# statgen/demuxlet

Measured on AMD Instinct MI355X. Metric: cell-SNP-sample triples/sec (singlet+doublet llk); HBM GB/s vs roofline, higher is better.
Workload: dtype f64

## Files before the change

demuxlet_amd/csrc/dmx_engine.hip:

```cpp
#include <hip/hip_runtime.h>

#include <algorithm>
#include <chrono>
#include <cmath>
#include <mutex>
#include <cstdlib>
#include <cstring>
#include <condition_variable>
#include <deque>
#include <new>
#include <memory>
#include <functional>
#include <thread>
#include <type_traits>
#include <unordered_map>
#include <cxxabi.h>
#include <string>
#include <numeric>
#include <vector>

#include "dmx_internal.hpp"
extern char** environ;
#include "dmx_log.hpp"
#include "dmx_engine_state.hpp"
// ... 3115 lines not shown
      DMX_WAVE_LDS_ORDER();
      const int cnt = (int)min<int64_t>(kTripPT, p_end - p0);
      for (int jj = 0; jj < cnt; jj += 2) {
        const int j = jj + h;
        const uint32_t nj = (ent && j < cnt) ? hdr[j].n : 0u;
        if (nj > 0) {
          const int64_t roff = hdr[j].off;
          uint32_t w = hdr[j].rd4;
          double f = s_pra[w & 0xFF][0] * qk + s_pra[w & 0xFF][1] * pk;
          int32_t E = 0;
          const bool deep = nj >= 8;
          for (uint32_t r = 1; r < nj; ++r) {
            if ((r & 3) == 0) w = load_rd4(pv, roff + r, nj - r);
            const uint32_t byte = (w >> (8 * (r & 3))) & 0xFF;
            f *= s_pra[byte][0] * qk + s_pra[byte][1] * pk;
            if (deep && (r & 7) == 7 && f < kAmbRescaleBelow && f > 0.0) {
              int e;
              (void)frexp(f, &e);
              f = ldexp(f, -e);
              E += e;
            }
          }
          const double wk = (double)hdr[j].gp[el] * (double)hdr[j].gp[3 + em];
          const double t = wk * f;
          st[j][k] = t;
          ste[j][k] = t > 0.0 ? E : kTripNoExp;
        }
      }
      DMX_WAVE_LDS_ORDER();
      if (fj < cnt && hdr[fj].n > 0) {
        int32_t En = kTripNoExp;
#pragma unroll
        for (int x = 0; x < 9; ++x) En = max(En, ste[fj][3 * x + fn]);
        if (En == kTripNoExp) En = 0;
        double u = 0.0;
#pragma unroll
        for (int x = 0; x < 9; ++x) {
          const double t = ldexp(st[fj][3 * x + fn], max(ste[fj][3 * x + fn] - En, -1100));
          u = x == 0 ? t : u + t;
        }
        su[fj][fn] = u;
        sue[fj][fn] = u > 0.0 ? En : kTripNoExp;
      }
      DMX_WAVE_LDS_ORDER();
      for (int j = 0; j < cnt; ++j) {
        const uint32_t nj = (uint32_t)__builtin_amdgcn_readfirstlane((int)hdr[j].n);
        if (nj == 0) continue;
        const int32_t snp = __builtin_amdgcn_readfirstlane(hdr[j].snp);
        const double u0 = amb_uniform(su[j][0]), u1 = amb_uniform(su[j][1]), u2 = amb_uniform(su[j][2]);
        const int32_t e0 = __builtin_amdgcn_readfirstlane(sue[j][0]), e1 = __builtin_amdgcn_readfirstlane(sue[j][1]),
                      e2 = __builtin_amdgcn_readfirstlane(sue[j][2]);
        const float* gs = g + (size_t)snp * V * 3;
#pragma unroll
        for (int a = 0; a < NACC; ++a) {
          const int32_t c = c0 + 64 * a;
          const float* gr = gs + (size_t)(c < V ? c : 0) * 3;
          const float g0 = gr[0], g1 = gr[1], g2 = gr[2];
          const bool nz = g0 != 0.f || g1 != 0.f || g2 != 0.f;
          double L;
          int32_t E = 0;
          if (nj < 8) {
            L = (double)g0 * u0 + (double)g1 * u1 + (double)g2 * u2;
          } else {
            E = kTripNoExp;
            if (g0 != 0.f) E = max(E, e0);
            if (g1 != 0.f) E = max(E, e1);
            if (g2 != 0.f) E = max(E, e2);
            if (E == kTripNoExp) E = 0;
            const double t0 = g0 != 0.f ? (double)g0 * ldexp(u0, max(e0 - E, -1100)) : 0.0;
            const double t1 = g1 != 0.f ? (double)g1 * ldexp(u1, max(e1 - E, -1100)) : 0.0;
            const double t2 = g2 != 0.f ? (double)g2 * ldexp(u2, max(e2 - E, -1100)) : 0.0;
            L = t0 + t1 + t2;
          }
          if (!nz) L = 1.0;
          double lg = dmx_log_is_special(L) ? log(L) : dmx_log_fast_pinned(L, s_log, lk);
          if (E != 0) lg = __builtin_fma((double)E, DMX_LOG_LN2HI, __builtin_fma((double)E, DMX_LOG_LN2LO, lg));
          if (nz) { acc[a] += lg; ns[a] += 1; nr[a] += (int32_t)nj; }
        }
      }
      DMX_WAVE_LDS_ORDER();
    }
  }
#pragma unroll
  for (int a = 0; a < NACC; ++a) {
    const int32_t c = c0 + 64 * a;
    if (c >= V) continue;
    ll[((size_t)slot * T + ti) * V + c] = acc[a];
    if (ti == 0) { n_snp[(size_t)slot * V + c] = ns[a]; n_read[(size_t)slot * V + c] = nr[a]; }
  }
}

__global__ void k_transpose_geno(const float* __restrict__ g, const double* __restrict__ gp0, int32_t S, int32_t V,
                                 float* __restrict__ gT, double* __restrict__ g0T) {
  const int nrow = V * 3;
  const int64_t n = (int64_t)S * nrow;
  for (int64_t i = (int64_t)blockIdx.x * blockDim.x + threadIdx.x; i < n; i += (int64_t)gridDim.x * blockDim.x) {
    const int64_t s = i % S;
    const int r = (int)(i / S);
    gT[i] = g[(size_t)s * nrow + r];
    if (r < 3) g0T[i] = gp0[(size_t)s * 3 + r];
  }
}

template <typename NRD, int NACC, bool FIXUP>
__global__ __launch_bounds__(kThreads) void k_doublet_generic(PileupView pv, const float* __restrict__ g,
                                                              const double* __restrict__ gp0,
                                                              const double* __restrict__ lut,
                                                              const double* __restrict__ alpha,
                                                              const int32_t* __restrict__ sched, int32_t V, int32_t A,
                                                              int32_t A_pad, int32_t TP, double* __restrict__ grid,
                                                              double* __restrict__ l00,
                                                              uint8_t* __restrict__ flagged) {
  if (FIXUP && !flags_any(flagged)) return;
  __shared__ double s_lut[kTab2];
  __shared__ double s_pG[kThreads * 9];
  __shared__ int32_t s_snp[32];
  __shared__ uint32_t s_cnt[32];
  __shared__ int64_t s_off[32];

  const int t = threadIdx.x;
  stage_k2_tables(s_lut, lut, t, kThreads);
  const double* s_log = s_lut + kLut2;
  for (int32_t bx = (int32_t)blockIdx.x; bx < pv.B; bx += (int32_t)gridDim.x) {
  if (FIXUP && !flagged[sched[bx]]) continue;
  const int32_t cell = sched[bx];
  const int64_t p_beg = pv.cell_pair_off[cell];
  const int64_t np = pv.cell_pair_off[cell + 1] - p_beg;
  int64_t rd_base = pv.cell_read_off[cell];
  const NRD* __restrict__ nrd = (const NRD*)pv.pair_nrd;

  const int ti1 = t / A_pad, n1 = t % A_pad;
  const bool lane1 = (ti1 < TP) && (n1 < A);
  double wA[9], wR[9];
  {
    const double al = lane1 ? alpha[n1] : 0.0;
#pragma unroll
    for (int l = 0; l < 3; ++l)
#pragma unroll
      for (int m = 0; m < 3; ++m) {
        const double p = 0.5 * l + (m - l) * 0.5 * al;
        wA[l * 3 + m] = p;
        wR[l * 3 + m] = 1.0 - p;
      }
  }

  const int32_t nAB = V * V * A;
  const int32_t nacc = nAB + A;
  const int32_t q0 = (int32_t)blockIdx.y * NACC * kThreads;
  bool ok = true;
  uint32_t code[NACC];
  double acc[NACC];
#pragma unroll
  for (int i = 0; i < NACC; ++i) {
    const int32_t q = q0 + t + i * kThreads;
    acc[i] = 0.0;
    if (q < nAB) {
      const int32_t n = q % A, jk = q / A;
      code[i] = ((uint32_t)(jk / V) << 20) | ((uint32_t)(jk % V) << 8) | (uint32_t)n;
    } else if (q < nacc) {
      code[i] = (0xFFFu << 20) | (uint32_t)(q - nAB);
    } else {
      code[i] = ~0u;
    }
  }
  __syncthreads();

  for (int64_t base = 0; base < np; base += TP) {
    const int tp = (int)min((int64_t)TP, np - base);
    if (t < 32) {
      const bool v = t < tp;
      const uint32_t n = v ? (uint32_t)nrd[p_beg + base + t] : 0u;
      uint32_t incl = n;
#pragma unroll
      for (int d = 1; d < 32; d <<= 1) {
        const uint32_t y = __shfl_up(incl, d, 32);
        if (t >= d) incl += y;
      }
      if (v) {
        s_cnt[t] = n;
        s_off[t] = rd_base + (int64_t)(incl - n);
        s_snp[t] = pv.pair_snp ? pv.pair_snp[p_beg + base + t] : (int32_t)(base + t);
      }
    }
    __syncthreads();
    rd_base = s_off[tp - 1] + (int64_t)s_cnt[tp - 1];

    {
      const bool on = lane1 && ti1 < tp;
      const uint32_t cnt = on ? s_cnt[ti1] : 0u;
      const int64_t off = on ? s_off[ti1] : 0;
      const uint32_t rd4 = load_rd4(pv, off, cnt);
      double pG[9];
      const double mx = pair_values_open<9, 0, true>(pv, cnt, off, rd4, s_lut, wA, wR, n1, pG, nullptr, on, A_pad);
      if (on) {
        const double y = rcp_refined(mx);
#pragma unroll
        for (int i = 0; i < 9; ++i) s_pG[(ti1 * A + n1) * 9 + i] = div_by(pG[i], mx, y);
      }
    }
    __syncthreads();

    for (int ti = 0; ti < tp; ++ti) {
      const int32_t snp = s_snp[ti];
      const float* __restrict__ grow = g + (size_t)snp * V * 3;
      const double* __restrict__ g0 = gp0 + (size_t)snp * 3;
#pragma unroll
      for (int i = 0; i < NACC; ++i) {
        const uint32_t cd = code[i];
        if (cd == ~0u) continue;
        const int32_t j = (cd >> 20) & 0xFFF, k = (cd >> 8) & 0xFFF, n = cd & 0xFF;
        double a[3], b[3];
        if (j == 0xFFF) {
          a[0] = b[0] = g0[0]; a[1] = b[1] = g0[1]; a[2] = b[2] = g0[2];
        } else {
          a[0] = (double)grow[j * 3]; a[1] = (double)grow[j * 3 + 1]; a[2] = (double)grow[j * 3 + 2];
          b[0] = (double)grow[k * 3]; b[1] = (double)grow[k * 3 + 1]; b[2] = (double)grow[k * 3 + 2];
        }
        const double* P = &s_pG[(ti * A + n) * 9];
        double sum = 0.0;
#pragma unroll
        for (int l = 0; l < 3; ++l)
#pragma unroll
          for (int m = 0; m < 3; ++m) sum += ((a[l] * b[m]) * P[l * 3 + m]);
        if (!FIXUP) ok &= __builtin_amdgcn_class(sum, 0x100);
        acc[i] += FIXUP ? log(sum) : dmx_log2_fast(sum, s_log);
      }
    }
    __syncthreads();
  }

#pragma unroll
  for (int i = 0; i < NACC; ++i) {
    const int32_t q = q0 + t + i * kThreads;
    if (q < nAB) grid[(size_t)cell * nAB + q] = acc[i];
    else if (q < nacc) l00[(size_t)cell * A + (q - nAB)] = acc[i];
  }
  if (!FIXUP && !ok) flag_cell(flagged, cell);
  __syncthreads();
  }
}

template <int TPC, int NK, int MINW, bool GD, bool CHK, int TP, bool SYMU>
__device__ __forceinline__ void a2_body(PileupView pv, int nrd_width, const float* __restrict__ g,
                                                         const double* __restrict__ gp0, const double* __restrict__ tabs,
                                                         const double* __restrict__ alpha,
                                                         const int32_t* __restrict__ sched, int32_t V, int32_t GS,
                                                         double* __restrict__ grid, double* __restrict__ l00,
                                                         uint8_t* __restrict__ flagged, const double* __restrict__ pfin, const double* __restrict__ pseed) {
  static_assert(!SYMU || ((TPC == 256 || TPC == 64) && NK == 4 && !CHK), "symmetric ownership: 32 samples on 256 threads or 16 on 64, eight accumulators per thread, provably safe rows");
  constexpr int kUV = TPC == 256 ? 32 : 16, kUSh = kUV == 32 ? 5 : 4;
  constexpr int A = 2;
  static_assert(TP == 32 || TP == 16 || TP == 8, "phase 1 runs on the first 2 * TP lanes of the cell's first wavefront");
  constexpr int CPW = kThreads / TPC;
  constexpr int T00 = TP + 2;
#define DMX_K2_SYNC() do { if (TPC == 64) { DMX_WAVE_LDS_ORDER(); } else { __syncthreads(); } } while (0)
  extern __shared__ __attribute__((aligned(16))) unsigned char s_raw[];
  __shared__ double s_tab[kTab2];
  __shared__ double s_w[2][18];
  const double* s_log = s_tab + kLut2;
  const int t = threadIdx.x;
  stage_k2_tables(s_tab, tabs, t, kThreads);
  if (t < 18) {
    const int n = t / 9, l = (t % 9) / 3, m = t % 3;
    const double p = 0.5 * l + (m - l) * 0.5 * alpha[n];
    s_w[n][t % 9] = p;
    s_w[n][9 + t % 9] = 1.0 - p;
  }
  __syncthreads();

  const int cw = t / TPC, tid = t % TPC;
  using g_t = typename std::conditional<GD, double, float>::type;
  const size_t cell_bytes = (size_t)TP * 18 * 8 + (size_t)TP * GS * sizeof(g_t) + 2 * T00 * 8 + TP * (4 + 4 + 8);
  unsigned char* base = s_raw + (size_t)cw * cell_bytes;
  double* s_pG = (double*)base;
  g_t* s_g = (g_t*)(base + (size_t)TP * 18 * 8);
  double* s_t00 = (double*)((unsigned char*)s_g + (size_t)TP * GS * sizeof(g_t));
  int64_t* s_off = (int64_t*)(s_t00 + 2 * T00);
  int32_t* s_snp = (int32_t*)(s_off + TP);
  uint32_t* s_cnt = (uint32_t*)(s_snp + TP);

  const int slot = blockIdx.x * CPW + cw;
  if (TPC == 64 && slot >= pv.B) return;
  const bool cell_ok = slot < pv.B;
  const int32_t cell = cell_ok ? sched[slot] : 0;
  const int64_t p_beg = cell_ok ? pv.cell_pair_off[cell] : 0;
  const int64_t np = cell_ok ? pv.cell_pair_off[cell + 1] - p_beg : 0;
  int64_t rd_base = cell_ok ? pv.cell_read_off[cell] : 0;

  const int KB = (V + NK - 1) / NK;
  const int JS = TPC / KB;
  const int jl = tid / KB, kb = tid % KB;
  const int j = (int)blockIdx.y * JS + jl;
  const bool owner = jl < JS && j < V;
  double acc[NK][A];
#pragma unroll
  for (int kk = 0; kk < NK; ++kk) { acc[kk][0] = 0.0; acc[kk][1] = 0.0; }
  bool ok = true;
  const DmxLogPins lk = dmx_log_pins();
  int uj[2] = {0, 0}, uk[2] = {0, 0};
  if constexpr (SYMU) {
#pragma unroll
    for (int su = 0; su < 2; ++su) { const int u = tid + TPC * su; uj[su] = u & (kUV - 1); uk[su] = (uj[su] + 1 + (u >> kUSh)) & (kUV - 1); }
  }
  const int ti1 = tid >> 1, n1 = tid & 1;
  double acc00 = 0.0;
  const int row_len = V * 3;

  for (int64_t tbase = 0; tbase < np; tbase += TP) {
    const int tp = (int)min((int64_t)TP, np - tbase);
    load_tile_headers<TP>(pv, nrd_width, p_beg, tbase, tp, tid, rd_base, s_cnt, s_off, s_snp);
    DMX_K2_SYNC();
    rd_base = s_off[tp - 1] + (int64_t)s_cnt[tp - 1];
    stage_geno_rows<TPC>(g, s_snp, tp, tid, row_len, GS, s_g);
    if (tid < 2 * TP) {
      const bool on = ti1 < tp;
      const uint32_t cnt = on ? s_cnt[ti1] : 0u;
      const int64_t off = on ? s_off[ti1] : 0;
      const uint32_t rd4 = load_rd4(pv, off, cnt);
      double vf[9];
      const int32_t fi = pfin ? certify_final_index(cnt, rd4) : -1;
      if (!__any(fi < 0)) {
        const double* fp = pfin + (size_t)fi * kCFinStride + (n1 ? 0 : 5);
        const double f0 = fp[0], f1 = fp[1], f2 = fp[2], f3 = n1 ? fp[3] : 0.0, f4 = n1 ? fp[4] : 0.0;
        const double f5[5] = {f0, f1, f2, f3, f4};
#pragma unroll
        for (int l = 0; l < 3; ++l)
#pragma unroll
          for (int m = 0; m < 3; ++m) vf[l * 3 + m] = n1 ? f5[l + m] : f5[l];
      } else if (pseed) {
        double q5[5], wA5[5], wR5[5];
#pragma unroll
        for (int q = 0; q < 5; ++q) {
          const int l = n1 ? (q > 2 ? 2 : q) : min(q, 2), m = n1 ? q - l : 0;
          const double p = 0.5 * l + (m - l) * 0.5 * (n1 ? 0.5 : 0.0);
          wA5[q] = p;
          wR5[q] = 1.0 - p;
        }
        certify_pair_values<5, false>(pv, cnt, off, rd4, s_tab, wA5, wR5, n1, q5, pseed);
#pragma unroll
        for (int l = 0; l < 3; ++l)
#pragma unroll
          for (int m = 0; m < 3; ++m) vf[l * 3 + m] = n1 ? q5[l + m] : q5[l];
      } else {
        double wA[9], wR[9];
#pragma unroll
        for (int i = 0; i < 9; ++i) { wA[i] = s_w[n1][i]; wR[i] = s_w[n1][9 + i]; }
        certify_pair_values<9, false, 2, true>(pv, cnt, off, rd4, s_tab, wA, wR, n1, vf);
      }
      if (on)
        ok &= llks00_term(gp0, s_snp[ti1], [&](int l, int m) { const double v = vf[l * 3 + m]; s_pG[(ti1 * 2 + n1) * 9 + l * 3 + m] = v; return v; },
                    s_log, &s_t00[n1 * T00 + ti1]);
    }
    DMX_K2_SYNC();
    if (tid < 2) {
      const double* row = &s_t00[tid * T00];
      if (tp == TP) {
        double2 v[TP / 2];
#pragma unroll
        for (int i = 0; i < TP / 2; ++i) v[i] = *reinterpret_cast<const double2*>(&row[2 * i]);
#pragma unroll
        for (int i = 0; i < TP / 2; ++i) { acc00 += v[i].x; acc00 += v[i].y; }
      } else {
        for (int i = 0; i < tp; ++i) acc00 += row[i];
      }
    }
    if constexpr (SYMU) {
      for (int ti = 0; ti < tp; ++ti) {
        const double* P = &s_pG[ti * 18];
        const double Q[3] = {P[0], P[3], P[6]};
        const double P1[5] = {P[9], P[10], P[11], P[14], P[17]};
        const g_t* gr = &s_g[ti * GS];
#pragma unroll
        for (int su = 0; su < 2; ++su) {
          const int js = uj[su], ks = uk[su];
          const double a[3] = {(double)gr[js * 3], (double)gr[js * 3 + 1], (double)gr[js * 3 + 2]};
          const double b[3] = {(double)gr[ks * 3], (double)gr[ks * 3 + 1], (double)gr[ks * 3 + 2]};
          double E[3][3];
#pragma unroll
          for (int l = 0; l < 3; ++l)
#pragma unroll
            for (int m = 0; m < 3; ++m) E[l][m] = a[l] * b[m];
          {
            double s_jk0 = E[0][0] * Q[0], s_kj0 = E[0][0] * Q[0];
#pragma unroll
            for (int l = 0; l < 3; ++l)
#pragma unroll
              for (int m = 0; m < 3; ++m) {
                if (l == 0 && m == 0) continue;
                s_jk0 += (E[l][m] * Q[l]);
                s_kj0 += (E[m][l] * Q[l]);
              }
            acc[2 * su][0] += dmx_log2_fast_pinned(s_jk0, s_log, lk);
            acc[2 * su + 1][0] += dmx_log2_fast_pinned(s_kj0, s_log, lk);
          }
          {
#pragma unroll
            for (int l = 0; l < 3; ++l)
#pragma unroll
              for (int m = 0; m < 3; ++m) E[l][m] = E[l][m] * P1[l + m];
            double s_jk1 = E[0][0], s_kj1 = E[0][0];
#pragma unroll
            for (int l = 0; l < 3; ++l)
#pragma unroll
              for (int m = 0; m < 3; ++m) {
                if (l == 0 && m == 0) continue;
                s_jk1 += E[l][m];
                s_kj1 += E[m][l];
              }
            acc[2 * su][1] += dmx_log2_fast_pinned(s_jk1, s_log, lk);
            acc[2 * su + 1][1] += dmx_log2_fast_pinned(s_kj1, s_log, lk);
          }
        }
      }
    } else
    if (owner) {
      for (int ti = 0; ti < tp; ++ti) {
        const double* P = &s_pG[ti * 18];
        double P0[9], P1[9];
#pragma unroll
        for (int i = 0; i < 9; ++i) { P0[i] = P[i]; P1[i] = P[9 + i]; }
        const g_t* gr = &s_g[ti * GS];
        const double a0 = (double)gr[j * 3], a1 = (double)gr[j * 3 + 1], a2 = (double)gr[j * 3 + 2];
        const double aj[3] = {a0, a1, a2};
#pragma unroll
        for (int kk = 0; kk < NK; ++kk) {
          const int k = min(kb * NK + kk, V - 1);
          const double b0 = (double)gr[k * 3], b1 = (double)gr[k * 3 + 1], b2 = (double)gr[k * 3 + 2];
          const double bk[3] = {b0, b1, b2};
          double s0 = (aj[0] * bk[0]) * P0[0], s1 = (aj[0] * bk[0]) * P1[0];
#pragma unroll
          for (int l = 0; l < 3; ++l)
#pragma unroll
            for (int m = 0; m < 3; ++m) {
              if (l == 0 && m == 0) continue;
              const double gp = aj[l] * bk[m];
              s0 += (gp * P0[l * 3 + m]);
              s1 += (gp * P1[l * 3 + m]);
            }
          if (CHK) ok &= __builtin_amdgcn_class(s0, 0x100) && __builtin_amdgcn_class(s1, 0x100);
          acc[kk][0] += dmx_log2_fast_pinned(s0, s_log, lk);
          acc[kk][1] += dmx_log2_fast_pinned(s1, s_log, lk);
        }
      }
    }
    DMX_K2_SYNC();
  }
  if (cell_ok) {
    if constexpr (SYMU) {
#pragma unroll
      for (int su = 0; su < 2; ++su) {
        const int u = tid + TPC * su, d = 1 + (u >> kUSh);
        if (d < kUV / 2 || (d == kUV / 2 && uj[su] < kUV / 2)) {
          double* o = grid + (((size_t)cell * V + uj[su]) * V + uk[su]) * A;
          o[0] = acc[2 * su][0]; o[1] = acc[2 * su][1];
          double* o2 = grid + (((size_t)cell * V + uk[su]) * V + uj[su]) * A;
          o2[0] = acc[2 * su + 1][0]; o2[1] = acc[2 * su + 1][1];
        }
      }
    } else
    if (owner) {
#pragma unroll
      for (int kk = 0; kk < NK; ++kk) {
        const int k = kb * NK + kk;
        if (k < V) {
          double* o = grid + (((size_t)cell * V + j) * V + k) * A;
          o[0] = acc[kk][0]; o[1] = acc[kk][1];
        }
      }
    }
    if (tid < 2 && blockIdx.y == 0) l00[(size_t)cell * A + tid] = acc00;
    if (!ok) flag_cell(flagged, cell);
  }
#undef DMX_K2_SYNC
}
template <int TPC, int NK, int MINW = 1, bool GD = false, bool CHK = true, int TP = 32>
__global__ __launch_bounds__(kThreads, (MINW == 1 && TPC == 64) ? 3 : MINW) void k_doublet_a2(PileupView pv, int nrd_width, const float* __restrict__ g,
                                                         const double* __restrict__ gp0, const double* __restrict__ tabs,
                                                         const double* __restrict__ alpha,
                                                         const int32_t* __restrict__ sched, int32_t V, int32_t GS,
                                                         double* __restrict__ grid, double* __restrict__ l00,
                                                         uint8_t* __restrict__ flagged, const double* __restrict__ pfin, const double* __restrict__ pseed) {
  a2_body<TPC, NK, MINW, GD, CHK, TP, false>(pv, nrd_width, g, gp0, tabs, alpha, sched, V, GS, grid, l00, flagged, pfin, pseed);
}
template <int MINW>
__global__ __launch_bounds__(kThreads, MINW) void k_doublet_a2u(PileupView pv, int nrd_width, const float* __restrict__ g,
                                                          const double* __restrict__ gp0, const double* __restrict__ tabs,
                                                          const double* __restrict__ alpha,
                                                          const int32_t* __restrict__ sched, int32_t V, int32_t GS,
                                                          double* __restrict__ grid, double* __restrict__ l00,
                                                          uint8_t* __restrict__ flagged, const double* __restrict__ pfin, const double* __restrict__ pseed) {
  a2_body<256, 4, MINW, true, false, 32, true>(pv, nrd_width, g, gp0, tabs, alpha, sched, V, GS, grid, l00, flagged, pfin, pseed);
}
__global__ __launch_bounds__(kThreads, 3) void k_doublet_a2u16(PileupView pv, int nrd_width, const float* __restrict__ g,
                                                          const double* __restrict__ gp0, const double* __restrict__ tabs,
                                                          const double* __restrict__ alpha,
                                                          const int32_t* __restrict__ sched, int32_t V, int32_t GS,
                                                          double* __restrict__ grid, double* __restrict__ l00,
                                                          uint8_t* __restrict__ flagged, const double* __restrict__ pfin, const double* __restrict__ pseed) {
  a2_body<64, 4, 1, false, false, 32, true>(pv, nrd_width, g, gp0, tabs, alpha, sched, V, GS, grid, l00, flagged, pfin, pseed);
}

template <int TPC, int NK>
__global__ __launch_bounds__(kThreads, 3) void k_doublet_a2f(PileupView pv, int nrd_width, const float* __restrict__ g,
                                                         const double* __restrict__ gp0, const double* __restrict__ tabs,
                                                         const double* __restrict__ alpha,
                                                         const int32_t* __restrict__ sched, int32_t V, int32_t GS,
                                                         double* __restrict__ grid, double* __restrict__ l00,
                                                         uint8_t* __restrict__ flagged) {
  constexpr int A = 2, TP = 32;
  constexpr int CPW = kThreads / TPC;
  constexpr int T00 = TP + 2;
#define DMX_K2_SYNC() do { if (TPC == 64) { DMX_WAVE_LDS_ORDER(); } else { __syncthreads(); } } while (0)
  extern __shared__ __attribute__((aligned(16))) unsigned char s_raw[];
  __shared__ double s_tab[kTab2];
  const double* s_log = s_tab + kLut2;
  const int t = threadIdx.x;
  stage_k2_tables(s_tab, tabs, t, kThreads);
  __syncthreads();

  const int cw = t / TPC, tid = t % TPC;
  constexpr bool SHARE = TPC > 64;
  constexpr int SUB = 8;
  const int VU = V;
  const size_t cell_bytes = (size_t)TP * 18 * 8 + (size_t)TP * GS * 4 + 2 * T00 * 8 + TP * (4 + 4 + 8) + (SHARE ? (size_t)SUB * 2 * VU * 32 : 0);
  unsigned char* base = s_raw + (size_t)cw * cell_bytes;
  double* s_pG = (double*)base;
  float* s_g = (float*)(base + (size_t)TP * 18 * 8);
  double* s_t00 = (double*)((unsigned char*)s_g + (size_t)TP * GS * 4);
  int64_t* s_off = (int64_t*)(s_t00 + 2 * T00);
  int32_t* s_snp = (int32_t*)(s_off + TP);
  uint32_t* s_cnt = (uint32_t*)(s_snp + TP);
  double* s_u = (double*)(s_cnt + TP);

  const int slot = blockIdx.x * CPW + cw;
  if (TPC == 64 && slot >= pv.B) return;
  const bool cell_ok = slot < pv.B;
  const int32_t cell = cell_ok ? sched[slot] : 0;
  const int64_t p_beg = cell_ok ? pv.cell_pair_off[cell] : 0;
  const int64_t np = cell_ok ? pv.cell_pair_off[cell + 1] - p_beg : 0;
  int64_t rd_base = cell_ok ? pv.cell_read_off[cell] : 0;

  const int KB = (V + NK - 1) / NK;
  const int JS = TPC / KB;
  const int jl = tid / KB, kb = tid % KB;
  const int j = (int)blockIdx.y * JS + jl;
  const bool owner = jl < JS && j < V;
  double acc[NK][A];
#pragma unroll
  for (int kk = 0; kk < NK; ++kk) { acc[kk][0] = 0.0; acc[kk][1] = 0.0; }
  bool ok = true;
  const DmxLogPins lk = dmx_log_pins();
  const int ti1 = tid >> 1, n1 = tid & 1;
  double wA[9], wR[9];
  {
    const double al = alpha[n1];
#pragma unroll
    for (int l = 0; l < 3; ++l)
#pragma unroll
      for (int m = 0; m < 3; ++m) {
        const double p = 0.5 * l + (m - l) * 0.5 * al;
        wA[l * 3 + m] = p;
        wR[l * 3 + m] = 1.0 - p;
      }
  }
  double acc00 = 0.0;
  const int row_len = V * 3;

  for (int64_t tbase = 0; tbase < np; tbase += TP) {
    const int tp = (int)min((int64_t)TP, np - tbase);
    load_tile_headers<TP>(pv, nrd_width, p_beg, tbase, tp, tid, rd_base, s_cnt, s_off, s_snp);
    DMX_K2_SYNC();
    rd_base = s_off[tp - 1] + (int64_t)s_cnt[tp - 1];
    stage_geno_rows<TPC>(g, s_snp, tp, tid, row_len, GS, s_g);
    if (tid < 64) {
      const bool on = ti1 < tp;
      const uint32_t cnt = on ? s_cnt[ti1] : 0u;
      const int64_t off = on ? s_off[ti1] : 0;
      const uint32_t rd4 = load_rd4(pv, off, cnt);
      double pG[9];
      const double mx = pair_values_open<9, 2, true>(pv, cnt, off, rd4, s_tab, wA, wR, n1, pG);
      if (on) {
        const double y = rcp_refined(mx);
        ok &= llks00_term(gp0, s_snp[ti1], [&](int l, int m) { const double v = div_by(pG[l * 3 + m], mx, y); s_pG[(ti1 * 2 + n1) * 9 + l * 3 + m] = v; return v; },
                    s_log, &s_t00[n1 * T00 + ti1]);
      }
    }
    DMX_K2_SYNC();
    if (tid < 2) {
      const double* row = &s_t00[tid * T00];
      if (tp == TP) {
        double2 v[TP / 2];
#pragma unroll
        for (int i = 0; i < TP / 2; ++i) v[i] = *reinterpret_cast<const double2*>(&row[2 * i]);
#pragma unroll
        for (int i = 0; i < TP / 2; ++i) { acc00 += v[i].x; acc00 += v[i].y; }
      } else {
        for (int i = 0; i < tp; ++i) acc00 += row[i];
      }
    }
    if (!SHARE) {
      if (owner) {
        for (int ti = 0; ti < tp; ++ti) {
          const double* P = &s_pG[ti * 18];
          double P0[9], P1[9];
#pragma unroll
          for (int i = 0; i < 9; ++i) { P0[i] = P[i]; P1[i] = P[9 + i]; }
          const float* gr = &s_g[ti * GS];
          const double a0 = (double)gr[j * 3], a1 = (double)gr[j * 3 + 1], a2 = (double)gr[j * 3 + 2];
#pragma unroll
          for (int kk = 0; kk < NK; ++kk) {
            const int k = min(kb * NK + kk, V - 1);
            const double b0 = (double)gr[k * 3], b1 = (double)gr[k * 3 + 1], b2 = (double)gr[k * 3 + 2];
            double x[3], y[3];
#pragma unroll
            for (int l = 0; l < 3; ++l) {
              x[l] = __builtin_fma(P0[l * 3 + 2], b2, __builtin_fma(P0[l * 3 + 1], b1, P0[l * 3] * b0));
              y[l] = __builtin_fma(P1[l * 3 + 2], b2, __builtin_fma(P1[l * 3 + 1], b1, P1[l * 3] * b0));
            }
            const double s0 = __builtin_fma(a2, x[2], __builtin_fma(a1, x[1], a0 * x[0]));
            const double s1 = __builtin_fma(a2, y[2], __builtin_fma(a1, y[1], a0 * y[0]));
            ok &= __builtin_amdgcn_class(s0, 0x100) && __builtin_amdgcn_class(s1, 0x100);
            acc[kk][0] += dmx_log2_fastmode(s0, s_log, lk);
            acc[kk][1] += dmx_log2_fastmode(s1, s_log, lk);
          }
        }
      }
      DMX_K2_SYNC();
    } else
#pragma unroll 1
    for (int sub = 0; sub < tp; sub += SUB) {
      const int ns = min(SUB, tp - sub);
#pragma unroll 1
      for (int e = tid; e < ns * 2 * V; e += TPC) {
        const int k = e % V, n = (e / V) & 1, pi = e / (2 * V);
        const double* P = &s_pG[((sub + pi) * 2 + n) * 9];
        const float* gr = &s_g[(sub + pi) * GS + k * 3];
        const double b0 = (double)gr[0], b1 = (double)gr[1], b2 = (double)gr[2];
        double* u = &s_u[(size_t)((pi * 2 + n) * VU + k) * 4];
#pragma unroll
        for (int l = 0; l < 3; ++l) u[l] = __builtin_fma(P[l * 3 + 2], b2, __builtin_fma(P[l * 3 + 1], b1, P[l * 3] * b0));
      }
      DMX_K2_SYNC();
      if (owner) {
#pragma unroll 1
        for (int pi = 0; pi < ns; ++pi) {
          const float* gr = &s_g[(sub + pi) * GS];
          const double a0 = (double)gr[j * 3], a1 = (double)gr[j * 3 + 1], a2 = (double)gr[j * 3 + 2];
          const double* u0 = &s_u[(size_t)((pi * 2 + 0) * VU) * 4];
          const double* u1 = &s_u[(size_t)((pi * 2 + 1) * VU) * 4];
#pragma unroll
          for (int kk = 0; kk < NK; ++kk) {
            const int k = min(kb * NK + kk, V - 1);
            const double2 x01 = *reinterpret_cast<const double2*>(&u0[k * 4]);
            const double x2 = u0[k * 4 + 2];
            const double2 y01 = *reinterpret_cast<const double2*>(&u1[k * 4]);
            const double y2 = u1[k * 4 + 2];
            const double s0 = __builtin_fma(a2, x2, __builtin_fma(a1, x01.y, a0 * x01.x));
            const double s1 = __builtin_fma(a2, y2, __builtin_fma(a1, y01.y, a0 * y01.x));
            ok &= __builtin_amdgcn_class(s0, 0x100) && __builtin_amdgcn_class(s1, 0x100);
            acc[kk][0] += dmx_log2_fastmode(s0, s_log, lk);
            acc[kk][1] += dmx_log2_fastmode(s1, s_log, lk);
          }
        }
      }
      DMX_K2_SYNC();
    }
    DMX_K2_SYNC();
  }
  if (cell_ok) {
    if (owner) {
#pragma unroll
      for (int kk = 0; kk < NK; ++kk) {
        const int k = kb * NK + kk;
        if (k < V) {
          double* o = grid + (((size_t)cell * V + j) * V + k) * A;
          o[0] = acc[kk][0]; o[1] = acc[kk][1];
        }
      }
    }
    if (tid < 2 && blockIdx.y == 0) l00[(size_t)cell * A + tid] = acc00;
    if (!ok) flag_cell(flagged, cell);
  }
#undef DMX_K2_SYNC
}

template <int TPC, int VMAX, int SUB, bool FIXJ, int MINW = 3, int NEP = 0, bool CHK = true>
__global__ __launch_bounds__(kThreads, MINW) void k_doublet_sym(PileupView pv, int nrd_width, const float* __restrict__ g,
                                                          const double* __restrict__ gp0, const double* __restrict__ tabs,
                                                          const int32_t* __restrict__ sched, int32_t V_and_flags,
                                                          double* __restrict__ grid, double* __restrict__ l00,
                                                          uint8_t* __restrict__ flagged, const double* __restrict__ pfin, const double* __restrict__ pseed) {
  const int32_t V = V_and_flags & 0xFFFF;
  const bool no_dma = (V_and_flags >> 16) & 1;
#if DMX_SYM_ABLATIONS
  const bool abl_p1 = (V_and_flags >> 17) & 1;
  const bool abl_p2 = (V_and_flags >> 18) & 1;
  const bool abl_u = (V_and_flags >> 19) & 1;
  const bool abl_00 = (V_and_flags >> 21) & 1;
#else
  constexpr bool abl_p1 = false, abl_p2 = false, abl_u = false, abl_00 = false;
#endif
  const bool no_prod = (V_and_flags >> 22) & 1;
  const bool no_pipe = (V_and_flags >> 23) & 1;
  const bool wait_all = (V_and_flags >> 24) & 1;
  static_assert(TPC == 16 || TPC == 32 || TPC == 64 || TPC == 256, "threads per barcode");
  constexpr int A = 2, TP = TPC >= 64 ? 32 : TPC / 2;
  static_assert(SUB <= TP && TP % 8 == 0, "sub-tile");
  constexpr int CPW = kThreads / TPC;
  constexpr int T00 = TP + 2;
  constexpr int NE = NEP ? NEP : (VMAX * (VMAX / 2 + 1) + VMAX + TPC - 1) / TPC;
  const int e_base = NEP ? (int)blockIdx.y * NEP * TPC : 0;
  constexpr int VUS = (VMAX + 2) & ~1;
  constexpr int GSS = (3 * VMAX + 3) & ~3;
#define DMX_K2_SYNC() do { if (TPC <= 64) { DMX_WAVE_LDS_ORDER(); } else { __syncthreads(); } } while (0)
// ... 6608 lines not shown
```

demuxlet_amd/csrc/dmx_log.hpp:

```cpp
#pragma once
#include <stdint.h>
#include <string.h>

#if defined(__HIPCC__)
#include <hip/hip_runtime.h>
#define DMX_HD __host__ __device__ __forceinline__
#else
#include <math.h>
#define DMX_HD static inline
#endif

#include "dmx_log_table.inc"

#define DMX_LOG_TABLE_DOUBLES 256
#define DMX_LOG2_TABLE_DOUBLES 512
#define DMX_LOG32_TABLE_DOUBLES 64

DMX_HD double dmx_log_core_comp(double x, uint32_t hi, uint32_t lo, const double* __restrict__ T) {
  const uint32_t tmp = hi - 0x3FE5F000u;
  const int32_t i = (int32_t)((tmp >> 13) & 127u);
  const int32_t k = (int32_t)tmp >> 20;
  const uint32_t zhi = hi - (tmp & 0xFFF00000u);
  const uint64_t zb = ((uint64_t)zhi << 32) | lo;
  double z;
  memcpy(&z, &zb, sizeof z);
  const double invc = T[2 * i], logc = T[2 * i + 1];
  const double r = __builtin_fma(z, invc, -1.0);
  const double kd = (double)k;
  const double w = __builtin_fma(kd, DMX_LOG_LN2HI, logc);
  const double h = w + r;
  double l = (w - h) + r;
  l = __builtin_fma(kd, DMX_LOG_LN2LO, l);
  const double r2 = r * r;
  double t1 = __builtin_fma(r, -0.25, 0x1.5555555555555p-2);
  double t2 = __builtin_fma(r, -0x1.5555555555555p-3, 0.2);
  t2 = __builtin_fma(r2, 0x1.2492492492492p-3, t2);
  t1 = __builtin_fma(r2, t2, t1);
  const double r3 = r * r2;
  double p = __builtin_fma(r3, t1, l);
  p = __builtin_fma(r2, -0.5, p);
  return p + h;
  (void)x;
}

DMX_HD double dmx_log_lite_core(uint32_t hi, uint32_t lo, const double* __restrict__ T) {
  const uint32_t tmp = hi - 0x3FE5F000u;
  const uint32_t k20 = tmp & 0xFFF00000u;
  const uint32_t zhi = hi - k20;
#if defined(__HIP_DEVICE_COMPILE__)
  const double z = __hiloint2double((int)zhi, (int)lo);
#else
  const uint64_t zb = ((uint64_t)zhi << 32) | lo;
  double z;
  memcpy(&z, &zb, sizeof z);
#endif
  const double* e = reinterpret_cast<const double*>(reinterpret_cast<const char*>(T) + ((tmp >> 9) & 0x7F0u));
  const double invc = e[0], logc = e[1];
  const double r = __builtin_fma(z, invc, -1.0);
  const double kd = (double)(int32_t)k20;
  const double w = __builtin_fma(kd, DMX_LOG_LN2HI * 0x1p-20, logc);
  const double r2 = r * r;
  double t1 = __builtin_fma(r, -0.25, 0x1.5555555555555p-2);
  double t2 = __builtin_fma(r, -0x1.5555555555555p-3, 0.2);
  t2 = __builtin_fma(r2, 0x1.2492492492492p-3, t2);
  t1 = __builtin_fma(r2, t2, t1);
  const double s = __builtin_fma(r, t1, -0.5);
  double p = __builtin_fma(r2, s, r);
  p = __builtin_fma(kd, DMX_LOG_LN2LO * 0x1p-20, p);
  return w + p;
}
DMX_HD double dmx_log2_core(uint32_t hi, uint32_t lo, const double* __restrict__ T) {
  const uint32_t tmp = hi - DMX_LOG2_OFF_HI;
  const uint32_t k20 = tmp & 0xFFF00000u;
  const uint32_t zhi = hi - k20;
#if defined(__HIP_DEVICE_COMPILE__)
  const double z = __hiloint2double((int)zhi, (int)lo);
#else
  const uint64_t zb = ((uint64_t)zhi << 32) | lo;
  double z;
  memcpy(&z, &zb, sizeof z);
#endif
  const double* e = reinterpret_cast<const double*>(reinterpret_cast<const char*>(T) + ((tmp >> 8) & 0xFF0u));
  const double invc = e[0], logc = e[1];
  const double r = __builtin_fma(z, invc, -1.0);
  const double kd = (double)(int32_t)k20;
  const double w = __builtin_fma(kd, DMX_LOG_LN2HI * 0x1p-20, logc);
  const double r2 = r * r;
  double t1 = __builtin_fma(r, -0.25, 0x1.5555555555555p-2);
  const double t2 = __builtin_fma(r, -0x1.5555555555555p-3, 0.2);
  t1 = __builtin_fma(r2, t2, t1);
  const double s = __builtin_fma(r, t1, -0.5);
  double p = __builtin_fma(r2, s, r);
  p = __builtin_fma(kd, DMX_LOG_LN2LO * 0x1p-20, p);
  return w + p;
}
DMX_HD double dmx_log2_lite32_core(uint32_t hi, uint32_t lo, const double* __restrict__ T32) {
  const uint32_t tmp = hi - DMX_LOG32_OFF_HI;
  const uint32_t k20 = tmp & 0xFFF00000u;
  const uint32_t zhi = hi - k20;
#if defined(__HIP_DEVICE_COMPILE__)
  const double z = __hiloint2double((int)zhi, (int)lo);
#else
  const uint64_t zb = ((uint64_t)zhi << 32) | lo;
  double z;
  memcpy(&z, &zb, sizeof z);
#endif
  const double* e = reinterpret_cast<const double*>(reinterpret_cast<const char*>(T32) + ((tmp >> 12) & 0xF8u));
  const double rc = e[0], logc = e[32];
  const double r = __builtin_fma(z, rc, -1.0);
  const double kd = (double)(int32_t)k20;
  const double w = __builtin_fma(kd, 0x1.62e42fefa39efp-1 * 0x1p-20, logc);
  double q = __builtin_fma(r, DMX_LOG32_A5, DMX_LOG32_A4);
  q = __builtin_fma(r, q, DMX_LOG32_A3);
  q = __builtin_fma(r, q, DMX_LOG32_A2);
  q = __builtin_fma(r, q, -0.5);
  q = __builtin_fma(r, q, 1.0);
  return __builtin_fma(r, q, w);
}
DMX_HD double dmx_log_core(double x, uint32_t hi, uint32_t lo, const double* __restrict__ T) {
  (void)x;
  return dmx_log_lite_core(hi, lo, T);
}

DMX_HD void dmx_log_dd(uint32_t hiw, uint32_t low, const double* __restrict__ T, const double* __restrict__ T2, double* out_hi, double* out_lo) {
  const uint32_t tmp = hiw - 0x3FE5F000u;
  const int32_t i = (int32_t)((tmp >> 13) & 127u);
  const int32_t k = (int32_t)tmp >> 20;
  const uint32_t zhi = hiw - (tmp & 0xFFF00000u);
#if defined(__HIP_DEVICE_COMPILE__)
  const double z = __hiloint2double((int)zhi, (int)low);
#else
  const uint64_t zb = ((uint64_t)zhi << 32) | low;
  double z;
  memcpy(&z, &zb, sizeof z);
#endif
  const double invc = T[2 * i], logc = T[2 * i + 1], logc_lo = T2[i];
  const double p = z * invc;
  const double pe = __builtin_fma(z, invc, -p);
  const double d = p - 1.0;
  const double rh = d + pe;
  const double rl = (d - rh) + pe;
  const double r2h = rh * rh;
  const double r2l = __builtin_fma(rh, rh, -r2h) + 2.0 * (rh * rl);
  double q = __builtin_fma(rh, -0.1, 0x1.c71c71c71c71cp-4);
  q = __builtin_fma(rh, q, -0.125);
  q = __builtin_fma(rh, q, 0x1.2492492492492p-3);
  q = __builtin_fma(rh, q, -0x1.5555555555555p-3);
  q = __builtin_fma(rh, q, 0.2);
  q = __builtin_fma(rh, q, -0.25);
  q = __builtin_fma(rh, q, 0x1.5555555555555p-2);
  const double t = (rh * r2h) * q;
  const double kd = (double)k;
  const double w = __builtin_fma(kd, DMX_LOG_LN2HI, logc);
  double s = w + rh, bb = s - w;
  const double e1 = (w - (s - bb)) + (rh - bb);
  const double a2 = -0.5 * r2h;
  double s2 = s + a2; bb = s2 - s;
  const double e2 = (s - (s2 - bb)) + (a2 - bb);
  double s3 = s2 + t; bb = s3 - s2;
  const double e3 = (s2 - (s3 - bb)) + (t - bb);
  const double a4 = kd * DMX_LOG_LN2LO;
  double s4 = s3 + a4; bb = s4 - s3;
  const double e4 = (s3 - (s4 - bb)) + (a4 - bb);
  const double tail = ((e1 + e2) + (e3 + e4)) + (((rl - 0.5 * r2l) + logc_lo) + kd * DMX_LOG_LN2LOLO);
  const double h = s4 + tail;
  *out_hi = h;
  *out_lo = (s4 - h) + tail;
}

DMX_HD void dmx_log_bracket(uint32_t hiw, uint32_t low, const double* __restrict__ T, const double* __restrict__ T2, double* t_lo, double* t_hi) {
  double h, l;
  dmx_log_dd(hiw, low, T, T2, &h, &l);
  *t_lo = h; *t_hi = h;
  if (l == 0.0 || h == 0.0) return;
  uint64_t hb;
  memcpy(&hb, &h, sizeof hb);
  const bool away = (l > 0.0) == (h > 0.0);
  const uint64_t nbits = away ? hb + 1 : hb - 1;
  double nb;
  memcpy(&nb, &nbits, sizeof nb);
  const double gap = nb - h;
  const double al = l < 0.0 ? -l : l, ag = gap < 0.0 ? -gap : gap;
  const bool near1 = (hiw - 0x3FEE0000u) < (0x3FF10900u - 0x3FEE0000u);
  if (al > (near1 ? 0.33 : 0.45) * ag) { if (nb < h) *t_lo = nb; else *t_hi = nb; }
}

#if defined(__HIPCC__)
__device__ __forceinline__ bool dmx_log_is_special(double x) { return !__builtin_amdgcn_class(x, 0x100); }
__device__ __forceinline__ double dmx_log_fast(double x, const double* __restrict__ T) {
  return dmx_log_core(x, (uint32_t)__double2hiint(x), (uint32_t)__double2loint(x), T);
}
__device__ __forceinline__ double dmx_log_lite(double x, const double* __restrict__ T) { return dmx_log_fast(x, T); }
struct DmxLogPins { double c13, c15, m14; };
__device__ __forceinline__ DmxLogPins dmx_log_pins() {
  DmxLogPins k{0x1.5555555555555p-2, 0.2, -0.25};
  asm volatile("" : "+v"(k.c13), "+v"(k.c15));
  asm volatile("" : "+s"(k.m14));
  return k;
}
__device__ __forceinline__ double dmx_log_fast_pinned(double x, const double* __restrict__ T, const DmxLogPins& K) {
  const uint32_t hi = (uint32_t)__double2hiint(x), lo = (uint32_t)__double2loint(x);
  const uint32_t tmp = hi - 0x3FE5F000u;
  const uint32_t k20 = tmp & 0xFFF00000u;
  const uint32_t zhi = hi - k20;
  const double z = __hiloint2double((int)zhi, (int)lo);
  const double* e = reinterpret_cast<const double*>(reinterpret_cast<const char*>(T) + ((tmp >> 9) & 0x7F0u));
  const double invc = e[0], logc = e[1];
  const double r = __builtin_fma(z, invc, -1.0);
  const double kd = (double)(int32_t)k20;
  const double w = __builtin_fma(kd, DMX_LOG_LN2HI * 0x1p-20, logc);
  const double r2 = r * r;
  double t1 = __builtin_fma(r, K.m14, K.c13);
  double t2 = __builtin_fma(r, -0x1.5555555555555p-3, K.c15);
  t2 = __builtin_fma(r2, 0x1.2492492492492p-3, t2);
  t1 = __builtin_fma(r2, t2, t1);
  const double s = __builtin_fma(r, t1, -0.5);
  double p = __builtin_fma(r2, s, r);
  p = __builtin_fma(kd, DMX_LOG_LN2LO * 0x1p-20, p);
  return w + p;
}
__device__ __forceinline__ double dmx_log2_fast(double x, const double* __restrict__ T) {
  return dmx_log2_core((uint32_t)__double2hiint(x), (uint32_t)__double2loint(x), T);
}
__device__ __forceinline__ double dmx_log2_fast_pinned(double x, const double* __restrict__ T, const DmxLogPins& K) {
  const uint32_t hi = (uint32_t)__double2hiint(x), lo = (uint32_t)__double2loint(x);
  const uint32_t tmp = hi - DMX_LOG2_OFF_HI;
  const uint32_t k20 = tmp & 0xFFF00000u;
  const uint32_t zhi = hi - k20;
  const double z = __hiloint2double((int)zhi, (int)lo);
  const double* e = reinterpret_cast<const double*>(reinterpret_cast<const char*>(T) + ((tmp >> 8) & 0xFF0u));
  const double invc = e[0], logc = e[1];
  const double r = __builtin_fma(z, invc, -1.0);
  const double kd = (double)(int32_t)k20;
  const double w = __builtin_fma(kd, DMX_LOG_LN2HI * 0x1p-20, logc);
  const double r2 = r * r;
  double t1 = __builtin_fma(r, K.m14, K.c13);
  const double t2 = __builtin_fma(r, -0x1.5555555555555p-3, K.c15);
  t1 = __builtin_fma(r2, t2, t1);
  const double s = __builtin_fma(r, t1, -0.5);
  double p = __builtin_fma(r2, s, r);
  p = __builtin_fma(kd, DMX_LOG_LN2LO * 0x1p-20, p);
  return w + p;
}
__device__ __forceinline__ double dmx_log2_lite(double x, const double* __restrict__ T, const DmxLogPins& K) {
  const uint32_t hi = (uint32_t)__double2hiint(x), lo = (uint32_t)__double2loint(x);
  const uint32_t tmp = hi - DMX_LOG2_OFF_HI;
  const uint32_t k20 = tmp & 0xFFF00000u;
  const uint32_t zhi = hi - k20;
  const double z = __hiloint2double((int)zhi, (int)lo);
  const double* e = reinterpret_cast<const double*>(reinterpret_cast<const char*>(T) + ((tmp >> 8) & 0xFF0u));
  const double invc = e[0], logc = e[1];
  const double r = __builtin_fma(z, invc, -1.0);
  const double kd = (double)(int32_t)k20;
  const double w = __builtin_fma(kd, 0x1.62e42fefa39efp-1 * 0x1p-20, logc);
  double q = __builtin_fma(r, K.m14, K.c13);
  q = __builtin_fma(r, q, -0.5);
  q = __builtin_fma(r, q, 1.0);
  return __builtin_fma(r, q, w);
}
struct DmxLog32Pins { double a5, a4, a3, a2; };
__device__ __forceinline__ DmxLog32Pins dmx_log32_pins() {
  DmxLog32Pins k{DMX_LOG32_A5, DMX_LOG32_A4, DMX_LOG32_A3, DMX_LOG32_A2};
  asm volatile("" : "+v"(k.a4));
  asm volatile("" : "+s"(k.a5), "+s"(k.a3), "+s"(k.a2));
  return k;
}
__device__ __forceinline__ double dmx_log2_lite32(double x, const double* __restrict__ T32, const DmxLog32Pins& K) {
  const uint32_t hi = (uint32_t)__double2hiint(x), lo = (uint32_t)__double2loint(x);
  const uint32_t tmp = hi - DMX_LOG32_OFF_HI;
  const uint32_t k20 = tmp & 0xFFF00000u;
  const uint32_t zhi = hi - k20;
  const double z = __hiloint2double((int)zhi, (int)lo);
  const double* e = reinterpret_cast<const double*>(reinterpret_cast<const char*>(T32) + ((tmp >> 12) & 0xF8u));
  const double rc = e[0], logc = e[32];
  const double r = __builtin_fma(z, rc, -1.0);
  const double kd = (double)(int32_t)k20;
  const double w = __builtin_fma(kd, 0x1.62e42fefa39efp-1 * 0x1p-20, logc);
  double q = __builtin_fma(r, K.a5, K.a4);
  q = __builtin_fma(r, q, K.a3);
  q = __builtin_fma(r, q, K.a2);
  q = __builtin_fma(r, q, -0.5);
  q = __builtin_fma(r, q, 1.0);
  return __builtin_fma(r, q, w);
}
__device__ __forceinline__ double dmx_log(double x, const double* __restrict__ T) {
  const double y = dmx_log_fast(x, T);
  return dmx_log_is_special(x) ? log(x) : y;
}
__device__ __forceinline__ void dmx_log_stage(double* s_tab, const double* __restrict__ g_tab, int tid, int nthreads) {
  for (int i = tid; i < DMX_LOG_TABLE_DOUBLES; i += nthreads) s_tab[i] = g_tab[i];
}
#else
static inline double dmx_log_comp_host_emul(double x) {
  uint64_t b;
  memcpy(&b, &x, sizeof b);
  const uint32_t hi = (uint32_t)(b >> 32), lo = (uint32_t)b;
  if ((hi - 0x00100000u) >= 0x7FE00000u) return log(x);
  return dmx_log_core_comp(x, hi, lo, dmx_log_table_host);
}
static inline double dmx_log2_host_emul(double x) {
  uint64_t b;
  memcpy(&b, &x, sizeof b);
  const uint32_t hi = (uint32_t)(b >> 32), lo = (uint32_t)b;
  if ((hi - 0x00100000u) >= 0x7FE00000u) return log(x);
  return dmx_log2_core(hi, lo, dmx_log2_table_host);
}
static inline double dmx_log2_lite32_host_emul(double x) {
  uint64_t b;
  memcpy(&b, &x, sizeof b);
  const uint32_t hi = (uint32_t)(b >> 32), lo = (uint32_t)b;
  if ((hi - 0x00100000u) >= 0x7FE00000u) return log(x);
  return dmx_log2_lite32_core(hi, lo, dmx_log32_table_host);
}
static inline double dmx_log_host_emul(double x) {
  uint64_t b;
  memcpy(&b, &x, sizeof b);
  const uint32_t hi = (uint32_t)(b >> 32), lo = (uint32_t)b;
  if ((hi - 0x00100000u) >= 0x7FE00000u) return log(x);
  return dmx_log_core(x, hi, lo, dmx_log_table_host);
}
#endif
```

Before: 14.26 billion.

## Software-pipeline LDS loads in symmetric doublet loop and split log2 table lookup

```diff
diff --git a/demuxlet_amd/csrc/dmx_engine.hip b/demuxlet_amd/csrc/dmx_engine.hip
--- a/demuxlet_amd/csrc/dmx_engine.hip
+++ b/demuxlet_amd/csrc/dmx_engine.hip
@@ -3441,6 +3441,8 @@
 #pragma unroll
     for (int su = 0; su < 2; ++su) { const int u = tid + TPC * su; uj[su] = u & (kUV - 1); uk[su] = (uj[su] + 1 + (u >> kUSh)) & (kUV - 1); }
   }
+  const g_t* const ga = s_g + uj[0] * 3;
+  const g_t* const gb[2] = {s_g + uk[0] * 3, s_g + uk[1] * 3};
   const int ti1 = tid >> 1, n1 = tid & 1;
   double acc00 = 0.0;
   const int row_len = V * 3;
@@ -3504,51 +3506,69 @@
       }
     }
     if constexpr (SYMU) {
-      for (int ti = 0; ti < tp; ++ti) {
-        const double* P = &s_pG[ti * 18];
-        const double Q[3] = {P[0], P[3], P[6]};
-        const double P1[5] = {P[9], P[10], P[11], P[14], P[17]};
-        const g_t* gr = &s_g[ti * GS];
+      const int tps = __builtin_amdgcn_readfirstlane(tp);
+      double Q[3], P1[5];
+      g_t ar[3], br[3];
+      auto load_pair = [&](int pi) {
+        const double* P = &s_pG[pi * 18];
+        Q[0] = P[0]; Q[1] = P[3]; Q[2] = P[6];
+        P1[0] = P[9]; P1[1] = P[10]; P1[2] = P[11]; P1[3] = P[14]; P1[4] = P[17];
+        const g_t* ra = &ga[pi * GS];
+        const g_t* rb = &gb[0][pi * GS];
+        ar[0] = ra[0]; ar[1] = ra[1]; ar[2] = ra[2];
+        br[0] = rb[0]; br[1] = rb[1]; br[2] = rb[2];
+      };
+      load_pair(0);
+      for (int ti = 0; ti < tps; ++ti) {
+        const double a[3] = {(double)ar[0], (double)ar[1], (double)ar[2]};
 #pragma unroll
         for (int su = 0; su < 2; ++su) {
-          const int js = uj[su], ks = uk[su];
-          const double a[3] = {(double)gr[js * 3], (double)gr[js * 3 + 1], (double)gr[js * 3 + 2]};
-          const double b[3] = {(double)gr[ks * 3], (double)gr[ks * 3 + 1], (double)gr[ks * 3 + 2]};
+          const double b[3] = {(double)br[0], (double)br[1], (double)br[2]};
           double E[3][3];
 #pragma unroll
           for (int l = 0; l < 3; ++l)
 #pragma unroll
             for (int m = 0; m < 3; ++m) E[l][m] = a[l] * b[m];
-          {
-            double s_jk0 = E[0][0] * Q[0], s_kj0 = E[0][0] * Q[0];
-#pragma unroll
-            for (int l = 0; l < 3; ++l)
-#pragma unroll
-              for (int m = 0; m < 3; ++m) {
-                if (l == 0 && m == 0) continue;
-                s_jk0 += (E[l][m] * Q[l]);
-                s_kj0 += (E[m][l] * Q[l]);
-              }
-            acc[2 * su][0] += dmx_log2_fast_pinned(s_jk0, s_log, lk);
-            acc[2 * su + 1][0] += dmx_log2_fast_pinned(s_kj0, s_log, lk);
+          double s_jk0 = E[0][0] * Q[0], s_kj0 = E[0][0] * Q[0];
+#pragma unroll
+          for (int l = 0; l < 3; ++l)
+#pragma unroll
+            for (int m = 0; m < 3; ++m) {
+              if (l == 0 && m == 0) continue;
+              s_jk0 += (E[l][m] * Q[l]);
+              s_kj0 += (E[m][l] * Q[l]);
+            }
+#pragma unroll
+          for (int l = 0; l < 3; ++l)
+#pragma unroll
+            for (int m = 0; m < 3; ++m) E[l][m] = E[l][m] * P1[l + m];
+          double s_jk1 = E[0][0], s_kj1 = E[0][0];
+#pragma unroll
+          for (int l = 0; l < 3; ++l)
+#pragma unroll
+            for (int m = 0; m < 3; ++m) {
+              if (l == 0 && m == 0) continue;
+              s_jk1 += E[l][m];
+              s_kj1 += E[m][l];
+            }
+          const DmxLog2Req r_jk0 = dmx_log2_request_fast(s_jk0, s_log), r_kj0 = dmx_log2_request_fast(s_kj0, s_log),
+                           r_jk1 = dmx_log2_request_fast(s_jk1, s_log), r_kj1 = dmx_log2_request_fast(s_kj1, s_log);
+          if (su == 0) {
+            const g_t* rb = &gb[1][ti * GS];
+            br[0] = rb[0]; br[1] = rb[1]; br[2] = rb[2];
           }
-          {
-#pragma unroll
-            for (int l = 0; l < 3; ++l)
-#pragma unroll
-              for (int m = 0; m < 3; ++m) E[l][m] = E[l][m] * P1[l + m];
-            double s_jk1 = E[0][0], s_kj1 = E[0][0];
-#pragma unroll
-            for (int l = 0; l < 3; ++l)
-#pragma unroll
-              for (int m = 0; m < 3; ++m) {
-                if (l == 0 && m == 0) continue;
-                s_jk1 += E[l][m];
-                s_kj1 += E[m][l];
-              }
-            acc[2 * su][1] += dmx_log2_fast_pinned(s_jk1, s_log, lk);
-            acc[2 * su + 1][1] += dmx_log2_fast_pinned(s_kj1, s_log, lk);
+          __builtin_amdgcn_sched_barrier(0);
+          __builtin_amdgcn_s_waitcnt(0xC07F);
+          __builtin_amdgcn_sched_barrier(0);
+          if (su == 1) {
+            load_pair(min(ti + 1, tps - 1));
+            __builtin_amdgcn_sched_barrier(0);
           }
+          acc[2 * su][0] += dmx_log2_finish_pinned(r_jk0, lk);
+          acc[2 * su + 1][0] += dmx_log2_finish_pinned(r_kj0, lk);
+          acc[2 * su][1] += dmx_log2_finish_pinned(r_jk1, lk);
+          acc[2 * su + 1][1] += dmx_log2_finish_pinned(r_kj1, lk);
+          __builtin_amdgcn_sched_barrier(0);
         }
       }
     } else
diff --git a/demuxlet_amd/csrc/dmx_log.hpp b/demuxlet_amd/csrc/dmx_log.hpp
--- a/demuxlet_amd/csrc/dmx_log.hpp
+++ b/demuxlet_amd/csrc/dmx_log.hpp
@@ -88,6 +88,36 @@
   const double r2 = r * r;
   double t1 = __builtin_fma(r, -0.25, 0x1.5555555555555p-2);
   const double t2 = __builtin_fma(r, -0x1.5555555555555p-3, 0.2);
+  t1 = __builtin_fma(r2, t2, t1);
+  const double s = __builtin_fma(r, t1, -0.5);
+  double p = __builtin_fma(r2, s, r);
+  p = __builtin_fma(kd, DMX_LOG_LN2LO * 0x1p-20, p);
+  return w + p;
+}
+struct DmxLog2Req { double z, invc, logc; int32_t k20; };
+DMX_HD DmxLog2Req dmx_log2_request(uint32_t hi, uint32_t lo, const double* __restrict__ T) {
+  const uint32_t tmp = hi - DMX_LOG2_OFF_HI;
+  const uint32_t k20 = tmp & 0xFFF00000u;
+  const uint32_t zhi = hi - k20;
+  DmxLog2Req q;
+#if defined(__HIP_DEVICE_COMPILE__)
+  q.z = __hiloint2double((int)zhi, (int)lo);
+#else
+  const uint64_t zb = ((uint64_t)zhi << 32) | lo;
+  memcpy(&q.z, &zb, sizeof q.z);
+#endif
+  const double* e = reinterpret_cast<const double*>(reinterpret_cast<const char*>(T) + ((tmp >> 8) & 0xFF0u));
+  q.invc = e[0]; q.logc = e[1];
+  q.k20 = (int32_t)k20;
+  return q;
+}
+DMX_HD double dmx_log2_finish(const DmxLog2Req& q, double c13, double c15, double m14) {
+  const double r = __builtin_fma(q.z, q.invc, -1.0);
+  const double kd = (double)q.k20;
+  const double w = __builtin_fma(kd, DMX_LOG_LN2HI * 0x1p-20, q.logc);
+  const double r2 = r * r;
+  double t1 = __builtin_fma(r, m14, c13);
+  const double t2 = __builtin_fma(r, -0x1.5555555555555p-3, c15);
   t1 = __builtin_fma(r2, t2, t1);
   const double s = __builtin_fma(r, t1, -0.5);
   double p = __builtin_fma(r2, s, r);
@@ -222,25 +252,12 @@
 __device__ __forceinline__ double dmx_log2_fast(double x, const double* __restrict__ T) {
   return dmx_log2_core((uint32_t)__double2hiint(x), (uint32_t)__double2loint(x), T);
 }
+__device__ __forceinline__ DmxLog2Req dmx_log2_request_fast(double x, const double* __restrict__ T) {
+  return dmx_log2_request((uint32_t)__double2hiint(x), (uint32_t)__double2loint(x), T);
+}
+__device__ __forceinline__ double dmx_log2_finish_pinned(const DmxLog2Req& q, const DmxLogPins& K) { return dmx_log2_finish(q, K.c13, K.c15, K.m14); }
 __device__ __forceinline__ double dmx_log2_fast_pinned(double x, const double* __restrict__ T, const DmxLogPins& K) {
-  const uint32_t hi = (uint32_t)__double2hiint(x), lo = (uint32_t)__double2loint(x);
-  const uint32_t tmp = hi - DMX_LOG2_OFF_HI;
-  const uint32_t k20 = tmp & 0xFFF00000u;
-  const uint32_t zhi = hi - k20;
-  const double z = __hiloint2double((int)zhi, (int)lo);
-  const double* e = reinterpret_cast<const double*>(reinterpret_cast<const char*>(T) + ((tmp >> 8) & 0xFF0u));
-  const double invc = e[0], logc = e[1];
-  const double r = __builtin_fma(z, invc, -1.0);
-  const double kd = (double)(int32_t)k20;
-  const double w = __builtin_fma(kd, DMX_LOG_LN2HI * 0x1p-20, logc);
-  const double r2 = r * r;
-  double t1 = __builtin_fma(r, K.m14, K.c13);
-  const double t2 = __builtin_fma(r, -0x1.5555555555555p-3, K.c15);
-  t1 = __builtin_fma(r2, t2, t1);
-  const double s = __builtin_fma(r, t1, -0.5);
-  double p = __builtin_fma(r2, s, r);
-  p = __builtin_fma(kd, DMX_LOG_LN2LO * 0x1p-20, p);
-  return w + p;
+  return dmx_log2_finish_pinned(dmx_log2_request_fast(x, T), K);
 }
 __device__ __forceinline__ double dmx_log2_lite(double x, const double* __restrict__ T, const DmxLogPins& K) {
   const uint32_t hi = (uint32_t)__double2hiint(x), lo = (uint32_t)__double2loint(x);
@@ -305,6 +322,14 @@
   if ((hi - 0x00100000u) >= 0x7FE00000u) return log(x);
   return dmx_log2_core(hi, lo, dmx_log2_table_host);
 }
+static inline double dmx_log2_split_host_emul(double x) {
+  uint64_t b;
+  memcpy(&b, &x, sizeof b);
+  const uint32_t hi = (uint32_t)(b >> 32), lo = (uint32_t)b;
+  if ((hi - 0x00100000u) >= 0x7FE00000u) return log(x);
+  const DmxLog2Req q = dmx_log2_request(hi, lo, dmx_log2_table_host);
+  return dmx_log2_finish(q, 0x1.5555555555555p-2, 0.2, -0.25);
+}
 static inline double dmx_log2_lite32_host_emul(double x) {
   uint64_t b;
   memcpy(&b, &x, sizeof b);
```

Result: faster. 14.57 billion (median of 6 runs) (+2.2%).
